# TheStageAI/TheWhisper

Hardware: NVIDIA H100
Metric: tokens_per_sec (higher is better)
Workload: dtype bf16

## Files before the change

### thewhisper_b200/csrc/api.cu

```cuda
#include <limits.h>
#include <stdarg.h>
#include <stdlib.h>
#include <string.h>

#include <map>
#include <string>
#include <tuple>
#include <vector>

#ifdef BW_F16
#define BW_RENAME_SUFFIX _f16
#define BW_API_NS bw_api_f16
#else
#define BW_RENAME_SUFFIX _bf16
#define BW_API_NS bw_api
#endif
#include "abi_rename.h"
#include "../../include/thewhisper_b200.h"
#include "decode.cuh"
#include "decode_mega_common.cuh"
#include "kernels.h"

namespace BW_NS {

// ... 217 lines not shown
constexpr int DPART_PER_ROW = 20480;

int step_batched_impl(bw_engine* e, cudaStream_t st);
int step_batched(bw_engine* e, cudaStream_t st) {
  if (g_pdl_enabled < 0) {
    const char* ev = getenv("BW_PDL");
    g_pdl_enabled = (ev && ev[0] == '0') ? 0 : 1;
  }
  g_pdl = g_pdl_enabled;
  const int rc = step_batched_impl(e, st);
  g_pdl = 0;
  return rc;
}
int step_batched_impl(bw_engine* e, cudaStream_t st) {
  const int D = e->D, H = e->H, S = e->S, ffn = e->cfg.ffn, Tmax = e->Tmax, Q = e->Q, A = e->A, G = e->G;
  const long long self_layer = (long long)e->cfg.max_audios * e->cfg.max_beams * Tmax * D;
  const long long cross_layer = (long long)e->cfg.max_audios * H * S * 64;
  const bool w8 = e->embed_scale != nullptr;
  auto proj = [&](const bf16* in, int K, const void* W, const float* sc, int N, int* ns) {
    const DecGemmPlan pl = gemm_dec_plan(Q, N, K, e->num_sms, true, w8);
    BW_CHECK((long long)pl.ksplit * N <= DPART_PER_ROW, "batched step: %d splits x N=%d exceed the partial-sum buffer", pl.ksplit, N);
    GemmEpi ep;
    ep.out_f32 = e->dpart; ep.row_stride = N;
    *ns = pl.ksplit;
    return gemm_dec(st, in, W, sc, Q, N, K, 0, ep, pl, (long long)Q * N);
  };
  if (int rc = launch_embed(st, e->embed, e->embed_scale, e->dec_pos, e->tokens, e->pos, e->dx, Q, D, Tmax)) return rc;
  int ns = 0;
  const float* pbias = nullptr;
  for (size_t l = 0; l < e->dec.size(); ++l) {
    const DecLayer& L = e->dec[l];
    bf16* kc = e->self_k + l * self_layer;
    bf16* vc = e->self_v + l * self_layer;
    if (int rc = launch_resid_ln(st, e->dx, e->dpart, ns, (long long)Q * D, pbias, L.ln1g, L.ln1b, e->dbn, Q, D)) return rc;
    if (int rc = proj(e->dbn, D, L.wqkv, L.sc[0], 3 * D, &ns)) return rc;
    {
      SelfAttnArgs s;
      s.qkv = e->dpart; s.nsplit = ns; s.split_stride = (long long)Q * 3 * D; s.qkv_bias = L.bqkv; s.q_alpha = 0.125f;
      s.kc = kc; s.vc = vc; s.kc_w = kc; s.vc_w = vc; s.anc = e->use_anc ? e->anc : nullptr; s.out_bf16 = e->dba; s.pos = e->pos;
      s.H = H; s.D = D; s.Tmax = Tmax;
      if (int rc = launch_self_attn(st, s, Q)) return rc;
    }
    if (int rc = proj(e->dba, D, L.wo, L.sc[1], D, &ns)) return rc;
    if (int rc = launch_resid_ln(st, e->dx, e->dpart, ns, (long long)Q * D, L.bo, L.ln2g, L.ln2b, e->dbn, Q, D)) return rc;
    if (int rc = proj(e->dbn, D, L.xwq, L.sc[2], D, &ns)) return rc;
    {
      CrossAttnArgs c;
      c.q = e->dpart; c.nsplit = ns; c.split_stride = (long long)Q * D; c.q_bias = L.xbq; c.q_alpha = 0.125f;
      c.kc = e->cross_k + l * cross_layer; c.vc = e->cross_v + l * cross_layer; c.out_bf16 = e->dba;
      c.part_o = e->part_o; c.part_ml = e->part_ml; c.counters = e->xcounters;
      c.S = S; c.H = H; c.D = D; c.G = G; c.pos = e->pos;
      if (e->opts.record_alignment && e->cfg.n_align_heads > 0) {
        c.align = e->align; c.head_slots = e->head_slots + l * H; c.Ha = e->cfg.n_align_heads;
        c.Tcap = e->cfg.max_align_steps; c.step_base = e->opts.begin_index;
      }
      if (int rc = launch_cross_attn(st, c, A)) return rc;
    }
    if (int rc = proj(e->dba, D, L.xwo, L.sc[3], D, &ns)) return rc;
    if (int rc = launch_resid_ln(st, e->dx, e->dpart, ns, (long long)Q * D, L.xbo, L.ln3g, L.ln3b, e->dbn, Q, D)) return rc;
    if (int rc = proj(e->dbn, D, L.w1, L.sc[4], ffn, &ns)) return rc;
    if (int rc = launch_gelu_bias(st, e->dpart, ns, (long long)Q * ffn, L.b1, e->dbh, Q, ffn)) return rc;
    if (int rc = proj(e->dbh, ffn, L.w2, L.sc[5], D, &ns)) return rc;
    pbias = L.b2;
  }
  if (int rc = launch_resid_ln(st, e->dx, e->dpart, ns, (long long)Q * D, pbias, e->dec_lnf_g, e->dec_lnf_b, e->dbn, Q, D)) return rc;
  {
    const DecGemmPlan pl = gemm_dec_plan(Q, e->V, D, e->num_sms, false, w8);
    GemmEpi ep;
    ep.out_f32 = e->logits; ep.row_stride = e->Vp;
    if (int rc = gemm_dec(st, e->dbn, e->embed, e->embed_scale, Q, e->V, D, e->V, ep, pl, 0)) return rc;
  }
  return 0;
}

constexpr int PREFILL_ROWS = 4096;

int prefill_pass(bw_engine* e, cudaStream_t st, int t0, int n) {
  const int D = e->D, H = e->H, S = e->S, ffn = e->cfg.ffn, Tmax = e->Tmax, Q = e->Q, R = e->Q * n;
  const long long self_layer = (long long)e->cfg.max_audios * e->cfg.max_beams * Tmax * D;
  const long long cross_layer = (long long)e->cfg.max_audios * H * S * 64;
  const bool w8 = e->embed_scale != nullptr;
  auto proj = [&](const bf16* in, int K, const void* W, const float* sc, int N, int* ns) {
    const DecGemmPlan pl = gemm_dec_plan(R, N, K, e->num_sms, true, w8);
    GemmEpi ep;
    ep.out_f32 = e->pf_part; ep.row_stride = N;
    *ns = pl.ksplit;
    return gemm_dec(st, in, W, sc, R, N, K, 0, ep, pl, (long long)R * N);
  };
  if (int rc = launch_prefill_embed(st, e->embed, e->embed_scale, e->dec_pos, e->tokens, e->pf_x, Q, n, t0, D, Tmax)) return rc;
  int ns = 0;
  const float* pbias = nullptr;
  for (size_t l = 0; l < e->dec.size(); ++l) {
    const DecLayer& L = e->dec[l];
    bf16* kc = e->self_k + l * self_layer;
    bf16* vc = e->self_v + l * self_layer;
    const bool last = l + 1 == e->dec.size();
    if (int rc = launch_resid_ln(st, e->pf_x, e->pf_part, ns, (long long)R * D, pbias, L.ln1g, L.ln1b, e->pf_n, R, D)) return rc;
    if (int rc = proj(e->pf_n, D, L.wqkv, L.sc[0], 3 * D, &ns)) return rc;
    if (int rc = launch_prefill_proj_sum(st, e->pf_part, ns, (long long)R * 3 * D, L.bqkv, 3 * D, D, R, last ? nullptr : e->pf_q, kc, vc, n,
                                         t0, Tmax))
      return rc;
    if (last) break;
    if (int rc = launch_prefill_self_attn(st, e->pf_q, kc, vc, e->pf_a, Q, n, t0, H, Tmax)) return rc;
    if (int rc = proj(e->pf_a, D, L.wo, L.sc[1], D, &ns)) return rc;
    if (int rc = launch_resid_ln(st, e->pf_x, e->pf_part, ns, (long long)R * D, L.bo, L.ln2g, L.ln2b, e->pf_n, R, D)) return rc;
    if (int rc = proj(e->pf_n, D, L.xwq, L.sc[2], D, &ns)) return rc;
    if (int rc = launch_prefill_proj_sum(st, e->pf_part, ns, (long long)R * D, L.xbq, D, D, R, e->pf_q, nullptr, nullptr, n, t0, Tmax)) return rc;
    if (int rc = launch_prefill_cross_attn(st, e->pf_q, e->cross_k + l * cross_layer, e->cross_v + l * cross_layer, e->pf_a, e->A, e->G, n, S, H))
      return rc;
    if (int rc = proj(e->pf_a, D, L.xwo, L.sc[3], D, &ns)) return rc;
    if (int rc = launch_resid_ln(st, e->pf_x, e->pf_part, ns, (long long)R * D, L.xbo, L.ln3g, L.ln3b, e->pf_n, R, D)) return rc;
    if (int rc = proj(e->pf_n, D, L.w1, L.sc[4], ffn, &ns)) return rc;
    if (int rc = launch_gelu_bias(st, e->pf_part, ns, (long long)R * ffn, L.b1, e->pf_h, R, ffn)) return rc;
    if (int rc = proj(e->pf_h, ffn, L.w2, L.sc[5], D, &ns)) return rc;
    pbias = L.b2;
  }
  return 0;
}

int prefill_fits(bw_engine* e, int R) {
  const int D = e->D, ffn = e->cfg.ffn;
  const int nk[4][2] = {{3 * D, D}, {D, D}, {ffn, D}, {D, ffn}};
  for (const auto& p : nk) {
    const DecGemmPlan pl = gemm_dec_plan(R, p[0], p[1], e->num_sms, true, e->embed_scale != nullptr);
    BW_CHECK((long long)pl.ksplit * R * p[0] <= e->pf_part_floats, "bw_decode_prefill: %d splits x %d rows x N=%d exceed the partial-sum buffer",
             pl.ksplit, R, p[0]);
  }
  return 0;
}

__global__ void set_pos_kernel(int* pos, int v) { *pos = v; }

int step_impl(bw_engine* e, cudaStream_t st) {
  const int D = e->D, H = e->H, S = e->S, ffn = e->cfg.ffn, V = e->V, Tmax = e->Tmax, Q = e->Q, A = e->A, G = e->G;
  const long long self_layer0 = (long long)e->cfg.max_audios * e->cfg.max_beams * Tmax * D;
  const long long cross_layer0 = (long long)e->cfg.max_audios * H * S * 64;
  bool mega_done = false, select_done = false;
  if (!e->no_mega && G == 1 && Q <= 8 && (int)e->dec.size() <= MEGA_MAXL) {
    MegaArgs m{};
    for (size_t l = 0; l < e->dec.size(); ++l) {
      const DecLayer& L = e->dec[l];
      MegaLayer& o = m.layers[l];
      o.ln1g = L.ln1g; o.ln1b = L.ln1b; o.bqkv = L.bqkv; o.bo = L.bo; o.ln2g = L.ln2g; o.ln2b = L.ln2b; o.xbq = L.xbq; o.xbo = L.xbo;
      o.ln3g = L.ln3g; o.ln3b = L.ln3b; o.b1 = L.b1; o.b2 = L.b2;
      o.wqkv = L.wqkv; o.wo = L.wo; o.xwq = L.xwq; o.xwo = L.xwo; o.w1 = L.w1; o.w2 = L.w2;
      o.self_k = e->self_k + l * self_layer0; o.self_v = e->self_v + l * self_layer0;
      o.cross_k = e->cross_k + l * cross_layer0; o.cross_v = e->cross_v + l * cross_layer0;
      o.head_slots = (e->opts.record_alignment && e->cfg.n_align_heads > 0) ? e->head_slots + l * H : nullptr;
    }
    m.L = (int)e->dec.size(); m.D = D; m.H = H; m.ffn = ffn; m.V = V; m.S = S; m.Tmax = Tmax; m.Q = Q;
    m.embed = e->embed; m.embed_scale = e->embed_scale; m.wscale = e->wscale_tab; m.dec_pos = e->dec_pos; m.lnf_g = e->dec_lnf_g; m.lnf_b = e->dec_lnf_b;
    m.tokens = e->tokens; m.pos = e->pos; m.ldl = e->Vp;
    m.dx = e->dx; m.dqkv = e->dqkv; m.dattn = e->dattn; m.dq = e->dq; m.dh = e->dh; m.logits = e->logits;
    m.part_o = e->part_o; m.part_ml = e->part_ml; m.xcounters = e->xcounters; m.bar = e->mega_bar;
    int ns = e->num_sms / (Q * H);
    const int ns_min = (S + 255) / 256;
    if (ns < ns_min) ns = ns_min;
    if (ns > XSPLIT) ns = XSPLIT;
    m.nsplit = ns;
    if (e->opts.record_alignment && e->cfg.n_align_heads > 0) {
      m.align = e->align; m.Ha = e->cfg.n_align_heads; m.Tcap = e->cfg.max_align_steps; m.step_base = e->opts.begin_index;
    }
    m.trace = e->mega_trace;
    if (!e->opts.timestamp_rules && !e->no_fused_select) {
      m.fuse_select = 1;
      m.suppress_bits = e->sup_bits; m.begin_suppress_bits = e->bsup_bits; m.begin_index = e->opts.begin_index;
      m.eos = e->opts.eos_token; m.pad = e->opts.pad_token; m.finished = e->finished; m.tokens_rw = e->tokens; m.pos_rw = e->pos;
      m.sel_best = e->sel_best; m.sel_ctr = e->sel_ctr;
    }
    m.flags = e->mega_flags;
    const int rc = launch_decode_mega(st, m, e->num_sms);
    if (rc == 0) {
      mega_done = true;
      select_done = m.fuse_select != 0;
    }
    else if (rc != -3) return rc;
  }
  if (!mega_done && !e->simt && Q >= e->batch_min) {
    if (int rc = step_batched(e, st)) return rc;
    mega_done = true;
  }
  if (!mega_done) {
  if (int rc = launch_embed(st, e->embed, e->embed_scale, e->dec_pos, e->tokens, e->pos, e->dx, Q, D, Tmax)) return rc;
  const long long self_layer = (long long)e->cfg.max_audios * e->cfg.max_beams * Tmax * D;
  const long long cross_layer = (long long)e->cfg.max_audios * H * S * 64;
  for (size_t l = 0; l < e->dec.size(); ++l) {
    const DecLayer& L = e->dec[l];
    bf16* kc = e->self_k + l * self_layer;
    bf16* vc = e->self_v + l * self_layer;
    for (int m0 = 0; m0 < Q; m0 += Q) {
      GemvArgs g;
      g.M = Q - m0;
      g.x = e->dx + (long long)m0 * D; g.ldx = D; g.ln_g = L.ln1g; g.ln_b = L.ln1b;
      g.W = L.wqkv; g.wscale = L.sc[0]; g.N = 3 * D; g.K = D; g.bias = L.bqkv; g.alpha = 0.125f; g.alpha_cols = D;
      g.out = e->dqkv + (long long)m0 * 3 * D; g.ldo = 3 * D;
      g.kc = kc; g.vc = vc; g.D = D; g.Tmax = Tmax; g.seq0 = m0; g.pos = e->pos;
      if (int rc = launch_gemv(st, g)) return rc;
    }
    {
      SelfAttnArgs s;
      s.qkv = e->dqkv; s.kc = kc; s.vc = vc; s.anc = e->use_anc ? e->anc : nullptr; s.out = e->dattn; s.pos = e->pos;
      s.H = H; s.D = D; s.Tmax = Tmax;
      if (int rc = launch_self_attn(st, s, Q)) return rc;
    }
    for (int m0 = 0; m0 < Q; m0 += Q) {
      GemvArgs g;
      g.M = Q - m0;
      g.x = e->dattn + (long long)m0 * D; g.ldx = D; g.W = L.wo; g.wscale = L.sc[1]; g.N = D; g.K = D; g.bias = L.bo;
      g.residual = e->dx + (long long)m0 * D; g.out = e->dx + (long long)m0 * D; g.ldo = D;
      if (int rc = launch_gemv(st, g)) return rc;
    }
    for (int m0 = 0; m0 < Q; m0 += Q) {
      GemvArgs g;
      g.M = Q - m0;
      g.x = e->dx + (long long)m0 * D; g.ldx = D; g.ln_g = L.ln2g; g.ln_b = L.ln2b;
      g.W = L.xwq; g.wscale = L.sc[2]; g.N = D; g.K = D; g.bias = L.xbq; g.alpha = 0.125f; g.alpha_cols = D;
      g.out = e->dq + (long long)m0 * D; g.ldo = D;
      if (int rc = launch_gemv(st, g)) return rc;
    }
    {
      CrossAttnArgs c;
      c.q = e->dq; c.kc = e->cross_k + l * cross_layer; c.vc = e->cross_v + l * cross_layer; c.out = e->dattn;
      c.part_o = e->part_o; c.part_ml = e->part_ml; c.counters = e->xcounters;
      c.S = S; c.H = H; c.D = D; c.G = G; c.pos = e->pos;
      if (e->opts.record_alignment && e->cfg.n_align_heads > 0) {
        c.align = e->align; c.head_slots = e->head_slots + l * H; c.Ha = e->cfg.n_align_heads;
        c.Tcap = e->cfg.max_align_steps; c.step_base = e->opts.begin_index;
      }
      if (int rc = launch_cross_attn(st, c, A)) return rc;
    }
    for (int m0 = 0; m0 < Q; m0 += Q) {
      GemvArgs g;
      g.M = Q - m0;
      g.x = e->dattn + (long long)m0 * D; g.ldx = D; g.W = L.xwo; g.wscale = L.sc[3]; g.N = D; g.K = D; g.bias = L.xbo;
      g.residual = e->dx + (long long)m0 * D; g.out = e->dx + (long long)m0 * D; g.ldo = D;
      if (int rc = launch_gemv(st, g)) return rc;
    }
    for (int m0 = 0; m0 < Q; m0 += Q) {
      GemvArgs g;
      g.M = Q - m0;
      g.x = e->dx + (long long)m0 * D; g.ldx = D; g.ln_g = L.ln3g; g.ln_b = L.ln3b;
      g.W = L.w1; g.wscale = L.sc[4]; g.N = ffn; g.K = D; g.bias = L.b1; g.act = 1;
      g.out = e->dh + (long long)m0 * ffn; g.ldo = ffn;
      if (int rc = launch_gemv(st, g)) return rc;
    }
    for (int m0 = 0; m0 < Q; m0 += Q) {
      GemvArgs g;
      g.M = Q - m0;
      g.x = e->dh + (long long)m0 * ffn; g.ldx = ffn; g.W = L.w2; g.wscale = L.sc[5]; g.N = D; g.K = ffn; g.bias = L.b2;
      g.residual = e->dx + (long long)m0 * D; g.out = e->dx + (long long)m0 * D; g.ldo = D;
      if (int rc = launch_gemv(st, g)) return rc;
    }
  }
  for (int m0 = 0; m0 < Q; m0 += Q) {
    GemvArgs g;
    g.M = Q - m0;
    g.x = e->dx + (long long)m0 * D; g.ldx = D; g.ln_g = e->dec_lnf_g; g.ln_b = e->dec_lnf_b;
    g.W = e->embed; g.wscale = e->embed_scale; g.N = V; g.K = D;
    g.out = e->logits + (long long)m0 * e->Vp; g.ldo = e->Vp;
    if (int rc = launch_gemv(st, g)) return rc;
  }
  }
  if (select_done) return 0;
  SelectArgs s;
  s.logits = e->logits; s.V = V; s.ldl = e->Vp; s.Q = Q; s.Tmax = Tmax; s.tokens = e->tokens; s.finished = e->finished; s.pos = e->pos;
  s.done_ctr = e->done_ctr; s.suppress_bits = e->sup_bits; s.begin_suppress_bits = e->bsup_bits;
  s.begin_index = e->opts.begin_index; s.eos = e->opts.eos_token; s.pad = e->opts.pad_token;
  s.ts_rules = e->opts.timestamp_rules; s.ts_begin = e->opts.timestamp_begin; s.no_ts = e->opts.no_timestamps_token;
  s.max_initial_ts = e->opts.max_initial_timestamp_index; s.out_lse = e->lse;
  if (G > 1) { s.n_cand = 2 * G; s.run_scores = e->run_scores; s.cand_scores = e->cand_scores; s.cand_tokens = e->cand_tokens; }
  return launch_select(st, s);
}

__global__ void mel_to_tm_kernel(const float* __restrict__ mel, bf16* __restrict__ out, int n_mels, int frames) {
  __shared__ float tile[32][33];
  const int b = blockIdx.z, f0 = blockIdx.x * 32, m0 = blockIdx.y * 32;
  const int tx = threadIdx.x & 31, ty = threadIdx.x >> 5;
  for (int i = ty; i < 32; i += 8) {
    const int m = m0 + i, f = f0 + tx;
    tile[i][tx] = (m < n_mels && f < frames) ? mel[((long long)b * n_mels + m) * frames + f] : 0.f;
  }
  __syncthreads();
  for (int i = ty; i < 32; i += 8) {
    const int f = f0 + i, m = m0 + tx;
    if (f < frames && m < n_mels) out[((long long)b * (frames + 2) + f + 1) * n_mels + m] = f2e(tile[tx][i]);
  }
}

__global__ void iota_anc_kernel(int* anc, int Q, int Tmax) {
  const int i = blockIdx.x * blockDim.x + threadIdx.x;
  if (i < Q * Tmax) anc[i] = i / Tmax;
}

__global__ void reorder_kernel(const int* __restrict__ anc_old, int* __restrict__ anc_new, const int* __restrict__ tok_old,
                               int* __restrict__ tok_new, const int* __restrict__ parent, const int* __restrict__ next_tok,
                               const int* __restrict__ pos_ptr, int Tmax) {
  const int i = blockIdx.x;
  const int p = parent[i];
  const int cur = *pos_ptr;
  for (int s = threadIdx.x; s < Tmax; s += blockDim.x) {
    anc_new[i * Tmax + s] = (s < cur) ? anc_old[p * Tmax + s] : i;
    int t = tok_old[p * Tmax + s];
    if (s == cur) t = next_tok[i];
    tok_new[i * Tmax + s] = t;
  }
}

// ... 633 lines not shown
```

### thewhisper_b200/csrc/decode.cuh

```cuda
#pragma once
#include "common.cuh"

namespace BW_NS {

struct GemvArgs {
  const float* x = nullptr;
  int ldx = 0;
  const float* ln_g = nullptr;
  const float* ln_b = nullptr;
  const void* W = nullptr;
  const float* wscale = nullptr;
  int N = 0, K = 0, M = 0;
  const float* bias = nullptr;
  float alpha = 1.0f;
  int alpha_cols = 0;
  int act = 0;
  const float* residual = nullptr;
  float* out = nullptr;
  int ldo = 0;
  bf16* kc = nullptr;
  bf16* vc = nullptr;
  int D = 0, Tmax = 0, seq0 = 0;
  const int* pos = nullptr;
};

struct SelfAttnArgs {
  const float* qkv = nullptr;
  const bf16* kc = nullptr;
  const bf16* vc = nullptr;
  const int* anc = nullptr;
  float* out = nullptr;
  bf16* out_bf16 = nullptr;
  const int* pos = nullptr;
  int H = 0, D = 0, Tmax = 0;
  bf16* kc_w = nullptr;
  bf16* vc_w = nullptr;
  int nsplit = 0;
  long long split_stride = 0;
  const float* qkv_bias = nullptr;
  float q_alpha = 1.0f;
};

constexpr int XSPLIT = 12;
constexpr int MAXG = 8;

struct CrossAttnArgs {
  const float* q = nullptr;
  const bf16* kc = nullptr;
  const bf16* vc = nullptr;
  float* out = nullptr;
  bf16* out_bf16 = nullptr;
  float* part_o = nullptr;
  float* part_ml = nullptr;
  unsigned* counters = nullptr;
  int S = 0, H = 0, D = 0, G = 1;
  float* align = nullptr;
  int align_slot = -1;
  const int* head_slots = nullptr;
  int Ha = 0, Tcap = 0, step_base = 0;
  const int* pos = nullptr;
  int nsplit = 0;
  long long split_stride = 0;
  const float* q_bias = nullptr;
  float q_alpha = 1.0f;
};

struct SelectArgs {
  const float* logits = nullptr;
  int V = 0, Q = 0, Tmax = 0, ldl = 0;
  int* tokens = nullptr;
  int* finished = nullptr;
  int* pos = nullptr;
  unsigned* done_ctr = nullptr;
  const unsigned* suppress_bits = nullptr;
  const unsigned* begin_suppress_bits = nullptr;
  int begin_index = 0;
  int eos = 0, pad = 0;
  int ts_rules = 0, ts_begin = 0, no_ts = 0, max_initial_ts = -1;
  float* out_lse = nullptr;
  int n_cand = 0;
  const float* run_scores = nullptr;
  float* cand_scores = nullptr;
  int* cand_tokens = nullptr;
};

struct MegaLayer {
  const float *ln1g, *ln1b, *bqkv, *bo, *ln2g, *ln2b, *xbq, *xbo, *ln3g, *ln3b, *b1, *b2;
  const void *wqkv, *wo, *xwq, *xwo, *w1, *w2;
  bf16 *self_k, *self_v;
  const bf16 *cross_k, *cross_v;
  const int* head_slots;
};

constexpr int MEGA_MAXL = 32;
constexpr int MEGA_DEFAULT_FLAGS = 64;
constexpr int MEGA_TRACE_N = 264;

struct MegaArgs {
  MegaLayer layers[MEGA_MAXL];
  int L, D, H, ffn, V, S, Tmax, Q;
  int ldl;
  const void* embed;
  const float* dec_pos;
  const float *lnf_g, *lnf_b;
  const int* tokens;
  const int* pos;
  float *dx, *dqkv, *dattn, *dq, *dh, *logits;
  float *part_o, *part_ml;
  unsigned* xcounters;
  unsigned* bar;
  int nsplit;
  float* align;
  int Ha, Tcap, step_base;
  long long* trace;
  int flags;
  int fuse_select;
  const unsigned* suppress_bits;
  const unsigned* begin_suppress_bits;
  int begin_index, eos, pad;
  int* finished;
  int* tokens_rw;
  int* pos_rw;
  unsigned long long* sel_best;
  unsigned* sel_ctr;
  int p0_off;
  const float* const* wscale;
  const float* embed_scale;
};

int launch_decode_mega(cudaStream_t st, const MegaArgs& a, int num_sms);
extern int g_mega_coop;
int launch_gemv(cudaStream_t st, const GemvArgs& a);
int launch_embed(cudaStream_t st, const void* E, const float* Es, const float* P, const int* tokens, const int* pos, float* x, int Q, int D, int Tmax);
int launch_self_attn(cudaStream_t st, const SelfAttnArgs& a, int Q);
int launch_cross_attn(cudaStream_t st, const CrossAttnArgs& a, int A);
int launch_select(cudaStream_t st, const SelectArgs& a);
int launch_resid_ln(cudaStream_t st, float* x, const float* part, int nsplit, long long split_stride, const float* bias, const float* g,
                    const float* b, bf16* y, int Q, int D);


int launch_prefill_embed(cudaStream_t st, const void* E, const float* Es, const float* P, const int* tokens, float* x, int Q, int n, int t0,
                         int D, int Tmax);
int launch_prefill_proj_sum(cudaStream_t st, const float* part, int nsplit, long long split_stride, const float* bias, int N, int D, int R,
                            bf16* qout, bf16* kc, bf16* vc, int n, int t0, int Tmax);
int launch_prefill_self_attn(cudaStream_t st, const bf16* q, const bf16* kc, const bf16* vc, bf16* out, int Q, int n, int t0, int H, int Tmax);
int launch_prefill_cross_attn(cudaStream_t st, const bf16* q, const bf16* kc, const bf16* vc, bf16* out, int A, int G, int n, int S, int H);

}
```

### thewhisper_b200/csrc/decode_mega.cu

```cuda
#include "decode_mega_common.cuh"

namespace BW_NS {

namespace {

using namespace mega;


constexpr unsigned V_NOTRACE = 1;

__device__ __noinline__ void wait_timeout(const char* what, unsigned a0, unsigned a1) {
  printf("[bw] decode_mega: %s timed out (block %d thread %d: %u %u)\n", what, blockIdx.x, threadIdx.x, a0, a1);
  __trap();
}
template <unsigned VAR>
struct GridBar {
  static constexpr bool TRACE = !(VAR & V_NOTRACE);
  unsigned* ctr;
  unsigned nblocks;
  unsigned epoch;
  long long* trace;
  __device__ __forceinline__ void arrive() {
    if (threadIdx.x == MT - 1) {
      if (TRACE && trace && epoch < MEGA_TRACE_N) trace[((long long)blockIdx.x * MEGA_TRACE_N + epoch) * 2] = global_ns();
      red_release_add(ctr, 1u);
    }
  }
  __device__ __forceinline__ void wait() {
    if (threadIdx.x == MT - 1) {
      const unsigned target = (epoch + 1) * nblocks;
      if (ld_acquire_u32(ctr) < target) {
        const long long t0 = clock64();
        while (ld_acquire_u32(ctr) < target) {
          if (clock64() - t0 > (1ll << 32)) {
            printf("[bw] decode_mega: grid barrier %u timed out (block %d)\n", epoch, blockIdx.x);
            __trap();
          }
        }
      }
      if (TRACE && trace && epoch < MEGA_TRACE_N) trace[((long long)blockIdx.x * MEGA_TRACE_N + epoch) * 2 + 1] = global_ns();
    }
    ++epoch;
    __syncthreads();
  }
  __device__ __forceinline__ void sync() {
    __syncthreads();
    arrive();
    wait();
  }
};

struct GemvDesc {
  const uint8_t* W;
  const float* scale;
  const float* bias;
  int N, K, R;
  int n0, nend;
  bool lm;
  const float* src;
  const float *lng, *lnb;
  float* out;
  int ldo;
  const float* residual;
  int act;
  float alpha;
  int alpha_cols;
  bf16 *kc, *vc;
};

__device__ __forceinline__ void split_rows(GemvDesc& d) {
  const int rc = (d.N + (int)gridDim.x - 1) / (int)gridDim.x;
  d.R = (rc + MW - 1) / MW;
  d.n0 = min(d.N, (int)blockIdx.x * rc);
  d.nend = min(d.N, d.n0 + rc);
}
template <unsigned VAR, bool W8>
__device__ __forceinline__ GemvDesc make_desc(const MegaArgs& a, const MegaLayer* layers, int l, int g, int pos) {
  GemvDesc d;
  d.scale = nullptr;
  if constexpr (W8) d.scale = l >= a.L ? a.embed_scale : a.wscale[l * 6 + g];
  d.lng = d.lnb = nullptr;
  d.residual = nullptr;
  d.act = 0;
  d.alpha = 1.f;
  d.alpha_cols = 0;
  d.kc = d.vc = nullptr;
  d.N = d.K = d.ldo = a.D;
  d.lm = false;
  if (l >= a.L) {
    d.W = static_cast<const uint8_t*>(a.embed); d.bias = nullptr; d.N = a.V; d.R = 2; d.n0 = 0; d.nend = a.V; d.lm = true; d.src = a.dx; d.lng = a.lnf_g; d.lnb = a.lnf_b; d.out = a.logits; d.ldo = a.ldl;
    return d;
  }
  const MegaLayer& L = layers[l];
  switch (g) {
    case 0:
      d.W = static_cast<const uint8_t*>(L.wqkv); d.bias = L.bqkv; d.N = 3 * a.D; d.src = a.dx; d.lng = L.ln1g; d.lnb = L.ln1b; d.out = a.dqkv; d.ldo = 3 * a.D;
      d.alpha = 0.125f; d.alpha_cols = a.D; d.kc = L.self_k; d.vc = L.self_v;
      break;
    case 1:
      d.W = static_cast<const uint8_t*>(L.wo); d.bias = L.bo; d.src = a.dattn; d.out = a.dx; d.residual = a.dx;
      break;
    case 2:
      d.W = static_cast<const uint8_t*>(L.xwq); d.bias = L.xbq; d.src = a.dx; d.lng = L.ln2g; d.lnb = L.ln2b; d.out = a.dq; d.alpha = 0.125f; d.alpha_cols = a.D;
      break;
    case 3:
      d.W = static_cast<const uint8_t*>(L.xwo); d.bias = L.xbo; d.src = a.dattn; d.out = a.dx; d.residual = a.dx;
      break;
    case 4:
      d.W = static_cast<const uint8_t*>(L.w1); d.bias = L.b1; d.N = a.ffn; d.src = a.dx; d.lng = L.ln3g; d.lnb = L.ln3b; d.out = a.dh; d.ldo = a.ffn; d.act = 1;
      break;
    default:
      d.W = static_cast<const uint8_t*>(L.w2); d.bias = L.b2; d.K = a.ffn; d.src = a.dh; d.out = a.dx; d.residual = a.dx;
      break;
  }
  split_rows(d);
  return d;
}

struct Pre {
  float bias;
  float scale;
  float4 g, b;
};

template <int ESZ>
__device__ __forceinline__ void issue_slabs(const GemvDesc& d, uint8_t* region, uint64_t* cbar) {
  if (threadIdx.x == DMA_T && d.n0 < d.nend) {
    const uint32_t bytes = (uint32_t)(d.nend - d.n0) * d.K * ESZ;
    mbar_arrive_expect_tx(cbar, bytes);
    if constexpr (ESZ == 2) bulk_g2s(region, reinterpret_cast<const bf16*>(d.W) + (long long)d.n0 * d.K, bytes, cbar);
    else bulk_g2s(region, d.W + (long long)d.n0 * d.K, bytes, cbar);
  }
}

template <bool W8>
__device__ __forceinline__ void prefetch_phase(const GemvDesc& d, Pre& p, uint8_t* pool, uint64_t* wbar, int gw, int warp, int lane) {
  constexpr int ESZ = W8 ? 1 : 2;
  int n;
  if (d.lm) {
    n = gw * d.R;
    if (n < d.N) issue_rows<ESZ>(pool + (size_t)warp * d.R * d.K * ESZ, wbar, d.W, d.K, d.R, n, d.N, lane);
  } else {
    n = d.n0 + warp * d.R;
  }
  const int r_sel = lane >> 3;
  p.bias = (d.bias && (lane & 7) < 2 && r_sel < d.R && n + r_sel < d.nend) ? d.bias[n + r_sel] : 0.f;
  if constexpr (W8) p.scale = (!d.lm && (lane & 7) < 2 && r_sel < d.R && n + r_sel < d.nend) ? d.scale[n + r_sel] : 1.f;
  const int k = threadIdx.x * 4;
  if (d.lng && k < d.K) {
    p.g = *reinterpret_cast<const float4*>(d.lng + k);
    p.b = *reinterpret_cast<const float4*>(d.lnb + k);
  }
}

__device__ __forceinline__ void stage_sync() { asm volatile("bar.sync 1, %0;" ::"n"(MT - 32) : "memory"); }
__device__ __forceinline__ void stage_done_stagers() {
  asm volatile("bar.sync 1, %0;" ::"n"(MT - 32) : "memory");
  asm volatile("bar.arrive 3, %0;" ::"n"(MT) : "memory");
}
__device__ __forceinline__ void stage_done_dma() { asm volatile("bar.sync 3, %0;" ::"n"(MT) : "memory"); }

template <int MB, unsigned VAR, class Dma>
__device__ __forceinline__ void stage_x(float* xs, float* red, const GemvDesc& d, const Pre& p, int M, bool split_end, Dma&& dma) {
  const int K = d.K;
  const int warp = threadIdx.x >> 5, lane = threadIdx.x & 31;
  if (warp == MW - 1) {
    dma();
    if (split_end) stage_done_dma();
    else __syncthreads();
    return;
  }
  constexpr int ST = MT - 32;
  if (!d.lng) {
    constexpr int U = 4;
    for (int base = threadIdx.x * 4; base < MB * K; base += ST * 4 * U) {
      float4 v[U];
#pragma unroll
      for (int u = 0; u < U; ++u) {
        const int i = base + u * ST * 4;
        const int m = (MB > 1 && i >= K) ? 1 : 0;
        v[u] = make_float4(0.f, 0.f, 0.f, 0.f);
        if (i < MB * K && m < M) v[u] = __ldcg(reinterpret_cast<const float4*>(d.src + (long long)m * K + (i - m * K)));
      }
#pragma unroll
      for (int u = 0; u < U; ++u) {
        const int i = base + u * ST * 4;
        if (i < MB * K) *reinterpret_cast<float4*>(xs + i) = v[u];
      }
    }
    if (split_end) stage_done_stagers();
    else __syncthreads();
    return;
  }
  const int k = threadIdx.x * 4;
  const bool have = k < K;
  float4 v[MB];
#pragma unroll
  for (int m = 0; m < MB; ++m) {
    v[m] = make_float4(0.f, 0.f, 0.f, 0.f);
    if (have && m < M) v[m] = __ldcg(reinterpret_cast<const float4*>(d.src + (long long)m * K + k));
  }
#pragma unroll
  for (int m = 0; m < MB; ++m) {
    const float s = warp_sum((v[m].x + v[m].y) + (v[m].z + v[m].w));
    if (lane == 0) red[m * MW + warp] = s;
  }
  stage_sync();
  float mean[MB];
#pragma unroll
  for (int m = 0; m < MB; ++m) {
    float s = 0.f;
#pragma unroll
    for (int w = 0; w < MW - 1; ++w) s += red[m * MW + w];
    mean[m] = s / (float)K;
    float ss = 0.f;
    if (have) {
      const float a0 = v[m].x - mean[m], a1 = v[m].y - mean[m], a2 = v[m].z - mean[m], a3 = v[m].w - mean[m];
      ss = (a0 * a0 + a1 * a1) + (a2 * a2 + a3 * a3);
    }
    ss = warp_sum(ss);
    if (lane == 0) red[(MB + m) * MW + warp] = ss;
  }
  stage_sync();
#pragma unroll
  for (int m = 0; m < MB; ++m) {
    float ss = 0.f;
#pragma unroll
    for (int w = 0; w < MW - 1; ++w) ss += red[(MB + m) * MW + w];
    const float rstd = rsqrtf(ss / (float)K + 1e-5f);
    if (have) {
      float4 o;
      o.x = (v[m].x - mean[m]) * rstd * p.g.x + p.b.x;
      o.y = (v[m].y - mean[m]) * rstd * p.g.y + p.b.y;
      o.z = (v[m].z - mean[m]) * rstd * p.g.z + p.b.z;
      o.w = (v[m].w - mean[m]) * rstd * p.g.w + p.b.w;
      *reinterpret_cast<float4*>(xs + m * K + k) = o;
    }
  }
  if (split_end) stage_done_stagers();
  else __syncthreads();
}

template <int MB, unsigned VAR, bool W8>
__device__ __forceinline__ void finish_rows(const GemvDesc& d, const float (&acc)[RMAX][MB], float scale, float bias, int n, int M,
                                            float res, bool res_valid, int D, int Tmax, int pos, int lane) {
  const int m = lane & 7, r_sel = lane >> 3;
  const int nn = n + r_sel;
  if (r_sel < d.R && m < MB && m < M && nn < d.nend) {
    float v = 0.f;
#pragma unroll
    for (int r = 0; r < RMAX; ++r) {
#pragma unroll
      for (int mm = 0; mm < MB; ++mm)
        if (r == r_sel && mm == m) v = acc[r][mm];
    }
    if (W8) v *= scale;
    v += bias;
    if (nn < d.alpha_cols) v *= d.alpha;
    if (d.act == 1) v = gelu_erf(v);
    if (d.residual) v += res_valid ? res : __ldcg(d.residual + (long long)m * d.ldo + nn);
    d.out[(long long)m * d.ldo + nn] = v;
    if (d.kc && nn >= D) {
      const long long row = ((long long)m * Tmax + pos) * D;
      if (nn < 2 * D) d.kc[row + nn - D] = f2e(v);
      else d.vc[row + nn - 2 * D] = f2e(v);
    }
  }
}

template <int MB, unsigned VAR, bool W8>
__global__ void __launch_bounds__(MT, 1) decode_mega_kernel(const __grid_constant__ MegaArgs a) {
  constexpr bool TRACE = !(VAR & V_NOTRACE);
  constexpr int ESZ = W8 ? 1 : 2;
  extern __shared__ __align__(128) uint8_t dyn[];
  float* red = reinterpret_cast<float*>(dyn);
  float* xs = red + 64;
  uint8_t* pool = reinterpret_cast<uint8_t*>(xs + (size_t)MB * a.ffn);
  uint8_t* att = pool + ATT_OFF;
  __shared__ unsigned s_last;
  __shared__ __align__(8) uint64_t wbar[2 * MW];
  __shared__ __align__(8) uint64_t xbar;
  __shared__ __align__(8) uint64_t cbar[2];
  __shared__ long long wts[MW][2];
  __shared__ __align__(16) MegaLayer sl[MEGA_MAXL];

  const int warp = threadIdx.x >> 5, lane = threadIdx.x & 31;
  const int gw = blockIdx.x * MW + warp, GW = gridDim.x * MW;
  const int D = a.D, H = a.H, Q = a.Q;
  const int pos0 = *a.pos;
  GridBar<VAR> bar{a.bar, gridDim.x, 0u, a.trace};
  const bool split_end = (a.flags & 64) != 0;
  long long* const mkbase = (TRACE && a.trace) ? a.trace + (long long)gridDim.x * MEGA_TRACE_N * 2 + (long long)blockIdx.x * MEGA_TRACE_N * 4 : nullptr;
  auto mark = [&](int j) {
    if (mkbase && threadIdx.x == 0 && bar.epoch < MEGA_TRACE_N) mkbase[bar.epoch * 4 + j] = global_ns();
  };

  const int nsplit = a.nsplit;
  const int ks = (a.S + nsplit - 1) / nsplit;
  const int grp = threadIdx.x >> 3, sub = threadIdx.x & 7;
  uint32_t wpar = 0, wpar1 = 0, xpar = 0, cpar0 = 0, cpar1 = 0;

  {
    static_assert(sizeof(MegaLayer) % 8 == 0, "MegaLayer is copied in 8-byte words");
    const unsigned long long* src = reinterpret_cast<const unsigned long long*>(a.layers);
    unsigned long long* dst = reinterpret_cast<unsigned long long*>(sl);
    for (int i = threadIdx.x; i < a.L * (int)(sizeof(MegaLayer) / 8); i += MT) dst[i] = src[i];
  }
  if (threadIdx.x == 0) {
    for (int i = 0; i < 2 * MW; ++i) mbar_init(&wbar[i], 1);
    mbar_init(&xbar, 1);
    mbar_init(&cbar[0], 1);
    mbar_init(&cbar[1], 1);
    fence_mbar_init();
  }
  __syncthreads();

  const int pos = pos0;
  GemvDesc cur = make_desc<VAR, W8>(a, sl, 0, 0, pos);
  Pre pre;
  const bool dbuf = a.p0_off > 0;
  issue_slabs<ESZ>(cur, pool + a.p0_off, &cbar[0]);
  prefetch_phase<W8>(cur, pre, pool, &wbar[warp], gw, warp, lane);
  if (blockIdx.x == 0) {
    for (int i = threadIdx.x; i < Q * D; i += MT) {
      const int q = i / D, d = i - q * D;
      const int tok = a.tokens[q * a.Tmax + pos];
      if constexpr (W8)
        a.dx[i] = a.embed_scale[tok] * (float)static_cast<const int8_t*>(a.embed)[(long long)tok * D + d] + a.dec_pos[(long long)pos * D + d];
      else
        a.dx[i] = e2f(static_cast<const bf16*>(a.embed)[(long long)tok * D + d]) + a.dec_pos[(long long)pos * D + d];
    }
  }
  bar.sync();

  const int nph = a.L * 6;
  for (int ph = 0; ph < nph; ++ph) {
    const int l = ph / 6, g = ph - l * 6;
    const MegaLayer& L = sl[l];
    {
      const int n = cur.n0 + warp * cur.R;
      const bool active = n < cur.nend;
      float res = 0.f;
      {
        const int m = lane & 7, r_sel = lane >> 3;
        if (cur.residual && active && r_sel < cur.R && m < MB && m < Q && n + r_sel < cur.nend)
          res = __ldcg(cur.residual + (long long)m * cur.ldo + n + r_sel);
      }
      auto ahead = [&]() {
        if (dbuf && ph + 1 < nph) {
          const GemvDesc d1 = make_desc<VAR, W8>(a, sl, (ph + 1) / 6, (ph + 1) % 6, pos);
          issue_slabs<ESZ>(d1, pool + (((ph + 1) & 1) ? 0 : a.p0_off), &cbar[(ph + 1) & 1]);
        }
        if (g == 0 && threadIdx.x == DMA_T + 1 && blockIdx.x < Q * H * nsplit) {
          const int item = blockIdx.x;
          const int split = item % nsplit, h = (item / nsplit) % H, q = item / (nsplit * H);
          const int s0 = split * ks;
          const int n = max(0, min(a.S, s0 + ks) - s0);
          if (n > 0) {
            l2_prefetch(L.cross_k + (((long long)q * H + h) * a.S + s0) * 64, (uint32_t)n * 128);
            l2_prefetch(L.cross_v + (((long long)q * H + h) * a.S + s0) * 64, (uint32_t)n * 128);
          }
        }
      };
      stage_x<MB, VAR>(xs, red, cur, pre, Q, split_end, ahead);
      mark(2);
      if (mkbase && lane == 0) wts[warp][0] = wts[warp][1] = 0;
      if (active) {
        mbar_wait(&cbar[ph & 1], (ph & 1) ? cpar1 : cpar0);
        if (mkbase && lane == 0) wts[warp][0] = global_ns();
        const uint8_t* slab = pool + ((ph & 1) ? 0 : a.p0_off) + (size_t)warp * cur.R * cur.K * ESZ;
        float acc[RMAX][MB];
        if (cur.R == 4) dot_rows<MB, 4, W8>(slab, xs, cur.K, acc, lane);
        else if (cur.R == 3) dot_rows<MB, 3, W8>(slab, xs, cur.K, acc, lane);
        else if (cur.R == 2) dot_rows<MB, 2, W8>(slab, xs, cur.K, acc, lane);
        else dot_rows<MB, 1, W8>(slab, xs, cur.K, acc, lane);
        finish_rows<MB, VAR, W8>(cur, acc, pre.scale, pre.bias, n, Q, res, true, D, a.Tmax, pos, lane);
        if (mkbase && lane == 0) wts[warp][1] = global_ns();
      }
      mark(3);
      if (cur.n0 < cur.nend) {
        if (ph & 1) cpar1 ^= 1u;
        else cpar0 ^= 1u;
      }
    }
    __syncthreads();
    bar.arrive();
    if (mkbase && threadIdx.x == 0 && bar.epoch < MEGA_TRACE_N) {
      long long t0 = 0, t1 = 0;
      for (int w = 0; w < MW; ++w) {
        t0 = wts[w][0] > t0 ? wts[w][0] : t0;
        t1 = wts[w][1] > t1 ? wts[w][1] : t1;
      }
      mkbase[bar.epoch * 4 + 0] = t0;
      mkbase[bar.epoch * 4 + 1] = t1;
    }
    cur = make_desc<VAR, W8>(a, sl, ph + 1 < nph ? (ph + 1) / 6 : a.L, (ph + 1) % 6, pos);
    if (!dbuf && !cur.lm) issue_slabs<ESZ>(cur, pool, &cbar[(ph + 1) & 1]);
    prefetch_phase<W8>(cur, pre, pool, &wbar[warp], gw, warp, lane);

    if (g == 0) {
      if (blockIdx.x < Q * H) {
        const int q = blockIdx.x / H, h = blockIdx.x - q * H;
        uint8_t* sK = att;
        uint8_t* sV = att + (size_t)MAXKEYS * 128;
        for (int s = grp; s < pos; s += KG) {
          const long long off = ((long long)q * a.Tmax + s) * D + h * 64 + sub * 8;
          cp_async16m(sK + s * 128 + sub * 16, L.self_k + off);
          cp_async16m(sV + s * 128 + sub * 16, L.self_v + off);
        }
      }
      bar.wait();
      for (int item = blockIdx.x; item < Q * H; item += gridDim.x) {
        const int q = item / H, h = item - q * H;
        const int n = pos + 1;
        uint8_t* sK = att;
        uint8_t* sV = att + (size_t)MAXKEYS * 128;
        float* redo = reinterpret_cast<float*>(att + (size_t)MAXKEYS * 256);
        const int s_first = (item == blockIdx.x) ? pos : 0;
        for (int s = s_first + grp; s < n; s += KG) {
          const long long off = ((long long)q * a.Tmax + s) * D + h * 64 + sub * 8;
          cp_async16m(sK + s * 128 + sub * 16, L.self_k + off);
          cp_async16m(sV + s * 128 + sub * 16, L.self_v + off);
        }
        float qv[8];
        {
          const float4 q0 = __ldcg(reinterpret_cast<const float4*>(a.dqkv + (long long)q * 3 * D + h * 64 + sub * 8));
          const float4 q1 = __ldcg(reinterpret_cast<const float4*>(a.dqkv + (long long)q * 3 * D + h * 64 + sub * 8 + 4));
          qv[0] = q0.x; qv[1] = q0.y; qv[2] = q0.z; qv[3] = q0.w; qv[4] = q1.x; qv[5] = q1.y; qv[6] = q1.z; qv[7] = q1.w;
        }
        cp_async_wait_allm();
        __syncthreads();
        float mx, sum, ov;
        if (n <= 3 * KG) attend_smem<3>(sK, sV, redo, red, qv, n, nullptr, mx, sum, ov);
        else attend_smem<(MAXKEYS + KG - 1) / KG>(sK, sV, redo, red, qv, n, nullptr, mx, sum, ov);
        if (threadIdx.x < 64) a.dattn[(long long)q * D + h * 64 + threadIdx.x] = ov / sum;
        fence_proxy_async_smem();
        __syncthreads();
      }
      bar.sync();
    } else if (g == 2) {
      if (threadIdx.x == 0 && blockIdx.x < Q * H * nsplit) {
        const int item = blockIdx.x;
        const int split = item % nsplit, h = (item / nsplit) % H, q = item / (nsplit * H);
        const int s0 = split * ks;
        const int n = max(0, min(a.S, s0 + ks) - s0);
        mbar_arrive_expect_tx(&xbar, (uint32_t)n * 256);
        if (n > 0) {
          bulk_g2s(att, L.cross_k + (((long long)q * H + h) * a.S + s0) * 64, (uint32_t)n * 128, &xbar);
          bulk_g2s(att + XKMAX * 128, L.cross_v + (((long long)q * H + h) * a.S + s0) * 64, (uint32_t)n * 128, &xbar);
        }
      }
      bar.wait();
      {
        uint8_t* sK = att;
        uint8_t* sV = att + XKMAX * 128;
        float* redo = reinterpret_cast<float*>(att + 2 * XKMAX * 128);
        for (int item = blockIdx.x; item < Q * H * nsplit; item += gridDim.x) {
          const int split = item % nsplit;
          const int h = (item / nsplit) % H;
          const int q = item / (nsplit * H);
          const int s0 = split * ks;
          const int n = max(0, min(a.S, s0 + ks) - s0);
          if (item != blockIdx.x && threadIdx.x == 0) {
            mbar_arrive_expect_tx(&xbar, (uint32_t)n * 256);
            if (n > 0) {
              bulk_g2s(sK, L.cross_k + (((long long)q * H + h) * a.S + s0) * 64, (uint32_t)n * 128, &xbar);
              bulk_g2s(sV, L.cross_v + (((long long)q * H + h) * a.S + s0) * 64, (uint32_t)n * 128, &xbar);
            }
          }
          float qv[8];
          {
            const float4 q0 = __ldcg(reinterpret_cast<const float4*>(a.dq + (long long)q * D + h * 64 + sub * 8));
            const float4 q1 = __ldcg(reinterpret_cast<const float4*>(a.dq + (long long)q * D + h * 64 + sub * 8 + 4));
            qv[0] = q0.x; qv[1] = q0.y; qv[2] = q0.z; qv[3] = q0.w; qv[4] = q1.x; qv[5] = q1.y; qv[6] = q1.z; qv[7] = q1.w;
          }
          float* align_row = nullptr;
          if (a.align && L.head_slots) {
            const int slot = L.head_slots[h];
            const int step = pos - a.step_base;
            if (slot >= 0 && step >= 0 && step < a.Tcap) align_row = a.align + (((long long)q * a.Ha + slot) * a.Tcap + step) * a.S + s0;
          }
          mbar_wait(&xbar, xpar);
          xpar ^= 1u;
          mark(0);
          if (mkbase && threadIdx.x == 0 && bar.epoch < MEGA_TRACE_N) mkbase[bar.epoch * 4 + 2] = clock64();
          float mx, sum, ov;
          attend_smem<(XKMAX + KG - 1) / KG>(sK, sV, redo, red, qv, n, align_row, mx, sum, ov,
                                             (mkbase && bar.epoch < MEGA_TRACE_N) ? mkbase + bar.epoch * 4 : nullptr);
          const long long pb = ((long long)q * H + h) * nsplit + split;
          if (threadIdx.x < 64) a.part_o[pb * 64 + threadIdx.x] = ov;
          if (threadIdx.x == 0) {
            a.part_ml[pb * 2 + 0] = mx;
            a.part_ml[pb * 2 + 1] = sum;
          }
          __syncthreads();
          if (threadIdx.x == 0) {
            const unsigned prev = atom_acq_rel_add(&a.xcounters[q * H + h], 1u);
            s_last = (prev == (unsigned)(nsplit - 1)) ? 1u : 0u;
          }
          __syncthreads();
          if (s_last && threadIdx.x < 64) {
            const long long hb = ((long long)q * H + h) * nsplit;
            float pm[XSPLIT], pl[XSPLIT], po[XSPLIT];
#pragma unroll
            for (int sp = 0; sp < XSPLIT; ++sp) {
              pm[sp] = -INFINITY; pl[sp] = 0.f; po[sp] = 0.f;
              if (sp < nsplit) {
                pm[sp] = __ldcg(&a.part_ml[(hb + sp) * 2]);
                pl[sp] = __ldcg(&a.part_ml[(hb + sp) * 2 + 1]);
                po[sp] = __ldcg(&a.part_o[(hb + sp) * 64 + threadIdx.x]);
              }
            }
            float M = -INFINITY;
#pragma unroll
            for (int sp = 0; sp < XSPLIT; ++sp)
              if (pl[sp] > 0.f) M = fmaxf(M, pm[sp]);
            float Lsum = 0.f, o = 0.f;
#pragma unroll
            for (int sp = 0; sp < XSPLIT; ++sp) {
              if (pl[sp] > 0.f) {
                const float w = __expf(pm[sp] - M);
                Lsum = fmaf(pl[sp], w, Lsum);
                o = fmaf(po[sp], w, o);
              }
            }
            a.dattn[(long long)q * D + h * 64 + threadIdx.x] = o / Lsum;
            if (threadIdx.x == 0) a.xcounters[q * H + h] = 0u;
          }
          fence_proxy_async_smem();
          __syncthreads();
        }
      }
      bar.sync();
    } else {
      bar.wait();
    }
  }

  stage_x<MB, VAR>(xs, red, cur, pre, Q, split_end, [] {});
  unsigned long long best = 0ull;
  {
    const int K = cur.K, N = cur.N;
    const size_t slab_bytes = (size_t)2 * K * ESZ;
    const size_t set_bytes = slab_bytes * MW;
    int buf = 0;
    const bool at_begin = (pos + 1 == a.begin_index) && a.begin_suppress_bits;
    for (int n = gw * 2; n < N; n += GW * 2) {
      const int n2 = n + GW * 2;
      if (n2 < N) {
        __syncwarp();
        issue_rows<ESZ>(pool + (buf ^ 1) * set_bytes + (size_t)warp * slab_bytes, &wbar[(buf ^ 1) * MW + warp], cur.W, K, 2, n2, N, lane);
      }
      float sc = 1.f;
      if constexpr (W8) sc = cur.scale[min(n + (lane >> 3), N - 1)];
      if (buf == 0) {
        mbar_wait(&wbar[warp], wpar);
        wpar ^= 1u;
      } else {
        mbar_wait(&wbar[MW + warp], wpar1);
        wpar1 ^= 1u;
      }
      float acc[RMAX][MB];
      dot_rows<MB, 2, W8>(pool + buf * set_bytes + (size_t)warp * slab_bytes, xs, K, acc, lane);
      finish_rows<MB, VAR, W8>(cur, acc, sc, 0.f, n, Q, 0.f, true, D, a.Tmax, pos, lane);
      if (a.fuse_select) {
        const int m = lane & 7, r_sel = lane >> 3, nn = n + r_sel;
        if (r_sel < 2 && m < MB && m < Q && nn < N) {
          float v = 0.f;
#pragma unroll
          for (int r = 0; r < 2; ++r)
#pragma unroll
            for (int mm = 0; mm < MB; ++mm)
              if (r == r_sel && mm == m) v = acc[r][mm];
          if (W8) v *= sc;
          bool masked = (a.suppress_bits[nn >> 5] >> (nn & 31)) & 1u;
          if (at_begin) masked = masked || ((a.begin_suppress_bits[nn >> 5] >> (nn & 31)) & 1u);
          if (!masked) {
            unsigned u = __float_as_uint(v);
            u = (u & 0x80000000u) ? ~u : (u | 0x80000000u);
            const unsigned long long key = ((unsigned long long)u << 32) | (unsigned long long)(0xffffffffu - (unsigned)nn);
            best = key > best ? key : best;
          }
        }
      }
      buf ^= 1;
    }
  }
  if (a.fuse_select) {
    {
      const unsigned long long o = __shfl_xor_sync(0xffffffffu, best, 8);
      best = o > best ? o : best;
    }
    unsigned long long* sb = reinterpret_cast<unsigned long long*>(xs);
    __syncthreads();
    if (lane < MB) sb[lane * MW + warp] = best;
    __syncthreads();
    if (threadIdx.x < MB && threadIdx.x < Q) {
      unsigned long long b = 0ull;
      for (int w = 0; w < MW; ++w) b = sb[threadIdx.x * MW + w] > b ? sb[threadIdx.x * MW + w] : b;
      if (b) atomicMax(a.sel_best + threadIdx.x, b);
    }
    __syncthreads();
    if (threadIdx.x == 0) {
      const unsigned prev = atom_acq_rel_add(a.sel_ctr, 1u);
      if (prev == gridDim.x - 1) {
        const int cur_len = pos + 1;
        const bool generating = cur_len >= a.begin_index && cur_len < a.Tmax;
        for (int q = 0; q < Q; ++q) {
          const unsigned long long b = __ldcg(a.sel_best + q);
          a.sel_best[q] = 0ull;
          if (generating) {
            int choice = (int)(0xffffffffu - (unsigned)(b & 0xffffffffull));
            if (a.finished[q]) choice = a.pad;
            else if (choice == a.eos) a.finished[q] = 1;
            a.tokens_rw[q * a.Tmax + cur_len] = choice;
          }
        }
        *a.sel_ctr = 0u;
        *a.pos_rw = pos + 1;
      }
    }
  }
  if (TRACE && a.trace && bar.epoch < MEGA_TRACE_N) {
    __syncthreads();
    if (threadIdx.x == 0) a.trace[((long long)blockIdx.x * MEGA_TRACE_N + bar.epoch) * 2] = global_ns();
  }
}

}

int g_mega_coop = -1;

namespace {

template <int MB, unsigned VAR, bool W8>
int launch_mega(cudaStream_t st, const MegaArgs& a, int num_sms, int coop) {
  static size_t limit = 0, attr = 0;
  if (!limit) {
    int dev = 0, optin = 0;
    BW_CUDA_OK(cudaGetDevice(&dev));
    BW_CUDA_OK(cudaDeviceGetAttribute(&optin, cudaDevAttrMaxSharedMemoryPerBlockOptin, dev));
    cudaFuncAttributes fa{};
    BW_CUDA_OK(cudaFuncGetAttributes(&fa, decode_mega_kernel<MB, VAR, W8>));
    limit = (size_t)optin - fa.sharedSizeBytes;
  }
  MegaArgs b = a;
  const size_t smem = mega_smem_plan(MB, a.D, a.ffn, num_sms, !(a.flags & 2), limit, &b.p0_off, W8 ? 1 : 2);
  if (!smem) return -3;
  if (smem > attr) {
    BW_CUDA_OK(cudaFuncSetAttribute(decode_mega_kernel<MB, VAR, W8>, cudaFuncAttributeMaxDynamicSharedMemorySize, (int)smem));
    int per_sm = 0;
    BW_CUDA_OK(cudaOccupancyMaxActiveBlocksPerMultiprocessor(&per_sm, decode_mega_kernel<MB, VAR, W8>, MT, smem));
    if (per_sm < 1) return -3;
    attr = smem;
  }
  BW_CUDA_OK(cudaMemsetAsync(a.bar, 0, 1024 * sizeof(unsigned), st));
  cudaLaunchConfig_t cfg{};
  cfg.gridDim = dim3(num_sms); cfg.blockDim = dim3(MT); cfg.dynamicSmemBytes = smem; cfg.stream = st;
  cudaLaunchAttribute at[1];
  at[0].id = cudaLaunchAttributeCooperative; at[0].val.cooperative = 1;
  cfg.attrs = at; cfg.numAttrs = coop ? 1 : 0;
  BW_CUDA_OK(cudaLaunchKernelEx(&cfg, decode_mega_kernel<MB, VAR, W8>, b));
  return 0;
}

}

int launch_decode_mega(cudaStream_t st, const MegaArgs& a, int num_sms) {
  const int Q = a.Q;
  const bool w8 = a.embed_scale != nullptr;
  const size_t esz = w8 ? 1 : 2;
  if (a.L > MEGA_MAXL || Q > 2 || a.D > MAXD || a.ffn > 5120 || a.D % 8 != 0 || a.ffn % 8 != 0 || a.Tmax > MAXKEYS) return -3;
  if ((size_t)MW * a.D * esz > (size_t)ATT_OFF) return -3;
  {
    const int nmax = 3 * a.D > a.ffn ? 3 * a.D : a.ffn;
    if (((nmax + num_sms - 1) / num_sms + MW - 1) / MW > RMAX) return -3;
  }
  if (a.nsplit > XSPLIT) return -3;
  if ((size_t)((a.D + num_sms - 1) / num_sms) * a.D * esz > (size_t)ATT_OFF) return -3;
  const int ks = (a.S + a.nsplit - 1) / a.nsplit;
  if (ks > XKMAX) return -3;
  int& coop = g_mega_coop;
  if (coop < 0) {
    const char* ev = getenv("BW_MEGA_COOP");
    coop = (ev && ev[0] == '0') ? 0 : 1;
  }
  int rc;
  if (w8) {
    if (Q <= 1) rc = a.trace ? launch_mega<1, 0u, true>(st, a, num_sms, coop) : launch_mega<1, V_NOTRACE, true>(st, a, num_sms, coop);
    else rc = a.trace ? launch_mega<2, 0u, true>(st, a, num_sms, coop) : launch_mega<2, V_NOTRACE, true>(st, a, num_sms, coop);
  } else {
    if (Q <= 1) rc = a.trace ? launch_mega<1, 0u, false>(st, a, num_sms, coop) : launch_mega<1, V_NOTRACE, false>(st, a, num_sms, coop);
// ... 9 lines not shown
```

Measured before the change: 813.8.

## Merge cross-attention split partials inside the output-projection staging step

Removes the atomic-counter, last-block split-KV merge from the cross-attention phase. The following output-projection GEMV now combines the per-split max/sum/output partials itself while staging its input vector, using warp shuffles across splits and float4 loads, and writes dattn only for its own column range. This drops two block barriers, an acquire-release atomic and a serialized tail merge per head. In exchange, every block repeats the merge for the full K when staging, and a named barrier is added between the DMA warp and the stagers.

```diff
diff --git a/thewhisper_b200/csrc/api.cu b/thewhisper_b200/csrc/api.cu
--- a/thewhisper_b200/csrc/api.cu
+++ b/thewhisper_b200/csrc/api.cu
@@ -393,7 +393,7 @@
     m.embed = e->embed; m.embed_scale = e->embed_scale; m.wscale = e->wscale_tab; m.dec_pos = e->dec_pos; m.lnf_g = e->dec_lnf_g; m.lnf_b = e->dec_lnf_b;
     m.tokens = e->tokens; m.pos = e->pos; m.ldl = e->Vp;
     m.dx = e->dx; m.dqkv = e->dqkv; m.dattn = e->dattn; m.dq = e->dq; m.dh = e->dh; m.logits = e->logits;
-    m.part_o = e->part_o; m.part_ml = e->part_ml; m.xcounters = e->xcounters; m.bar = e->mega_bar;
+    m.part_o = e->part_o; m.part_ml = e->part_ml; m.bar = e->mega_bar;
     int ns = e->num_sms / (Q * H);
     const int ns_min = (S + 255) / 256;
     if (ns < ns_min) ns = ns_min;
diff --git a/thewhisper_b200/csrc/decode.cuh b/thewhisper_b200/csrc/decode.cuh
--- a/thewhisper_b200/csrc/decode.cuh
+++ b/thewhisper_b200/csrc/decode.cuh
@@ -107,7 +107,6 @@
   const int* pos;
   float *dx, *dqkv, *dattn, *dq, *dh, *logits;
   float *part_o, *part_ml;
-  unsigned* xcounters;
   unsigned* bar;
   int nsplit;
   float* align;
diff --git a/thewhisper_b200/csrc/decode_mega.cu b/thewhisper_b200/csrc/decode_mega.cu
--- a/thewhisper_b200/csrc/decode_mega.cu
+++ b/thewhisper_b200/csrc/decode_mega.cu
@@ -104,7 +104,7 @@
       d.W = static_cast<const uint8_t*>(L.xwq); d.bias = L.xbq; d.src = a.dx; d.lng = L.ln2g; d.lnb = L.ln2b; d.out = a.dq; d.alpha = 0.125f; d.alpha_cols = a.D;
       break;
     case 3:
-      d.W = static_cast<const uint8_t*>(L.xwo); d.bias = L.xbo; d.src = a.dattn; d.out = a.dx; d.residual = a.dx;
+      d.W = static_cast<const uint8_t*>(L.xwo); d.bias = L.xbo; d.src = a.part_o; d.out = a.dx; d.residual = a.dx;
       break;
     case 4:
       d.W = static_cast<const uint8_t*>(L.w1); d.bias = L.b1; d.N = a.ffn; d.src = a.dx; d.lng = L.ln3g; d.lnb = L.ln3b; d.out = a.dh; d.ldo = a.ffn; d.act = 1;
@@ -153,6 +153,69 @@
   }
 }
 
+template <int MB>
+__device__ __forceinline__ void merge_xattn(float* xs, const GemvDesc& d, const MegaArgs& a, int M) {
+  constexpr int XC = 6;
+  static_assert(MAXD <= (MT - 32) * 4 && XSPLIT <= 16, "one float4 per staging thread and sequence; one lane per split");
+  const int K = d.K, nsplit = a.nsplit;
+  const int k = threadIdx.x * 4, sp_l = threadIdx.x & 15;
+  const bool have = k < K;
+#pragma unroll 1
+  for (int m = 0; m < MB; ++m) {
+    const int hb = (m * a.H + (k >> 6)) * nsplit;
+    const float* po_base = a.part_o + hb * 64 + (k & 63);
+    const bool live = have && m < M;
+    float pm = -INFINITY, pl = 0.f;
+    float4 po[XC];
+    if (live && sp_l < nsplit) {
+      const float2 v = __ldcg(reinterpret_cast<const float2*>(a.part_ml) + hb + sp_l);
+      pm = v.x;
+      pl = v.y;
+    }
+#pragma unroll
+    for (int sp = 0; sp < XC; ++sp) {
+      po[sp] = make_float4(0.f, 0.f, 0.f, 0.f);
+      if (live && sp < nsplit) po[sp] = __ldcg(reinterpret_cast<const float4*>(po_base + sp * 64));
+    }
+    if (m == 0) asm volatile("bar.arrive 2, %0;" ::"n"(MT) : "memory");
+    float mx = pl > 0.f ? pm : -INFINITY;
+#pragma unroll
+    for (int s = 8; s >= 1; s >>= 1) mx = fmaxf(mx, __shfl_xor_sync(0xffffffffu, mx, s));
+    float lsum = 0.f;
+    float4 o = make_float4(0.f, 0.f, 0.f, 0.f);
+    for (int sp0 = 0;;) {
+#pragma unroll
+      for (int sp = 0; sp < XC; ++sp) {
+        const float sm = __shfl_sync(0xffffffffu, pm, sp0 + sp, 16), sl = __shfl_sync(0xffffffffu, pl, sp0 + sp, 16);
+        if (sp0 + sp < nsplit && sl > 0.f) {
+          const float w = __expf(sm - mx);
+          lsum = fmaf(sl, w, lsum);
+          o.x = fmaf(po[sp].x, w, o.x);
+          o.y = fmaf(po[sp].y, w, o.y);
+          o.z = fmaf(po[sp].z, w, o.z);
+          o.w = fmaf(po[sp].w, w, o.w);
+        }
+      }
+      sp0 += XC;
+      if (sp0 >= nsplit) break;
+#pragma unroll
+      for (int sp = 0; sp < XC; ++sp)
+        if (live && sp0 + sp < nsplit) po[sp] = __ldcg(reinterpret_cast<const float4*>(po_base + (sp0 + sp) * 64));
+    }
+    if (!have) continue;
+    float4 v = make_float4(0.f, 0.f, 0.f, 0.f);
+    if (m < M) {
+      v = make_float4(o.x / lsum, o.y / lsum, o.z / lsum, o.w / lsum);
+      float* row = a.dattn + m * K;
+      if (k >= d.n0 && k < d.nend) row[k] = v.x;
+      if (k + 1 >= d.n0 && k + 1 < d.nend) row[k + 1] = v.y;
+      if (k + 2 >= d.n0 && k + 2 < d.nend) row[k + 2] = v.z;
+      if (k + 3 >= d.n0 && k + 3 < d.nend) row[k + 3] = v.w;
+    }
+    *reinterpret_cast<float4*>(xs + m * K + k) = v;
+  }
+}
+
 __device__ __forceinline__ void stage_sync() { asm volatile("bar.sync 1, %0;" ::"n"(MT - 32) : "memory"); }
 __device__ __forceinline__ void stage_done_stagers() {
   asm volatile("bar.sync 1, %0;" ::"n"(MT - 32) : "memory");
@@ -161,12 +224,20 @@
 __device__ __forceinline__ void stage_done_dma() { asm volatile("bar.sync 3, %0;" ::"n"(MT) : "memory"); }
 
 template <int MB, unsigned VAR, class Dma>
-__device__ __forceinline__ void stage_x(float* xs, float* red, const GemvDesc& d, const Pre& p, int M, bool split_end, Dma&& dma) {
+__device__ __forceinline__ void stage_x(float* xs, float* red, const GemvDesc& d, const Pre& p, int M, bool split_end, const MegaArgs& a,
+                                        bool xattn, Dma&& dma) {
   const int K = d.K;
   const int warp = threadIdx.x >> 5, lane = threadIdx.x & 31;
   if (warp == MW - 1) {
+    if (xattn) asm volatile("bar.sync 2, %0;" ::"n"(MT) : "memory");
     dma();
     if (split_end) stage_done_dma();
+    else __syncthreads();
+    return;
+  }
+  if (xattn) {
+    merge_xattn<MB>(xs, d, a, M);
+    if (split_end) stage_done_stagers();
     else __syncthreads();
     return;
   }
@@ -277,7 +348,6 @@
   float* xs = red + 64;
   uint8_t* pool = reinterpret_cast<uint8_t*>(xs + (size_t)MB * a.ffn);
   uint8_t* att = pool + ATT_OFF;
-  __shared__ unsigned s_last;
   __shared__ __align__(8) uint64_t wbar[2 * MW];
   __shared__ __align__(8) uint64_t xbar;
   __shared__ __align__(8) uint64_t cbar[2];
@@ -362,7 +432,7 @@
           }
         }
       };
-      stage_x<MB, VAR>(xs, red, cur, pre, Q, split_end, ahead);
+      stage_x<MB, VAR>(xs, red, cur, pre, Q, split_end, a, g == 3, ahead);
       mark(2);
       if (mkbase && lane == 0) wts[warp][0] = wts[warp][1] = 0;
       if (active) {
@@ -493,40 +563,6 @@
             a.part_ml[pb * 2 + 0] = mx;
             a.part_ml[pb * 2 + 1] = sum;
           }
-          __syncthreads();
-          if (threadIdx.x == 0) {
-            const unsigned prev = atom_acq_rel_add(&a.xcounters[q * H + h], 1u);
-            s_last = (prev == (unsigned)(nsplit - 1)) ? 1u : 0u;
-          }
-          __syncthreads();
-          if (s_last && threadIdx.x < 64) {
-            const long long hb = ((long long)q * H + h) * nsplit;
-            float pm[XSPLIT], pl[XSPLIT], po[XSPLIT];
-#pragma unroll
-            for (int sp = 0; sp < XSPLIT; ++sp) {
-              pm[sp] = -INFINITY; pl[sp] = 0.f; po[sp] = 0.f;
-              if (sp < nsplit) {
-                pm[sp] = __ldcg(&a.part_ml[(hb + sp) * 2]);
-                pl[sp] = __ldcg(&a.part_ml[(hb + sp) * 2 + 1]);
-                po[sp] = __ldcg(&a.part_o[(hb + sp) * 64 + threadIdx.x]);
-              }
-            }
-            float M = -INFINITY;
-#pragma unroll
-            for (int sp = 0; sp < XSPLIT; ++sp)
-              if (pl[sp] > 0.f) M = fmaxf(M, pm[sp]);
-            float Lsum = 0.f, o = 0.f;
-#pragma unroll
-            for (int sp = 0; sp < XSPLIT; ++sp) {
-              if (pl[sp] > 0.f) {
-                const float w = __expf(pm[sp] - M);
-                Lsum = fmaf(pl[sp], w, Lsum);
-                o = fmaf(po[sp], w, o);
-              }
-            }
-            a.dattn[(long long)q * D + h * 64 + threadIdx.x] = o / Lsum;
-            if (threadIdx.x == 0) a.xcounters[q * H + h] = 0u;
-          }
           fence_proxy_async_smem();
           __syncthreads();
         }
@@ -537,7 +573,7 @@
     }
   }
 
-  stage_x<MB, VAR>(xs, red, cur, pre, Q, split_end, [] {});
+  stage_x<MB, VAR>(xs, red, cur, pre, Q, split_end, a, false, [] {});
   unsigned long long best = 0ull;
   {
     const int K = cur.K, N = cur.N;
```

Result: faster. 850.5, median of 6 (+4.5%).
